# sqliteai/sqlite-vector

Hardware: AMD Instinct MI355X
Metric: vectors scanned/sec, L2 top-20 over Nx384 f32 (higher is better)
Workload: dtype f32; 1 GPU; 10Mx384 f32 L2 top-20 single-query; rows_per_gpu=10000000, dim=384, k=20, backend=HIP gfx950 x1

## Files before the change

### sqlite-vector_amd/csrc/vg_corpus.hip

```cpp
#include "vg_internal.h"

#include <atomic>
#include <mutex>
#include <utility>
#include <vector>

#include "vg_device.h"


static thread_local std::string g_err;

int vg_fail(int code, const char *fmt, ...) {
    char buf[1024];
    va_list ap;
    va_start(ap, fmt);
    vsnprintf(buf, sizeof(buf), fmt, ap);
    va_end(ap);
    g_err = buf;
    return code;
}

extern "C" const char *vg_last_error(void) { return g_err.c_str(); }
extern "C" void vg_set_last_error_(const char *msg) { g_err = msg ? msg : ""; }

// ... 70 lines not shown
    {"VG_SHAPE_F16_ROUND3", 1},
    {"VG_SHAPE_INT_SHORT_ROUND3", 1},
    {"VG_SHAPE_PREF_ROUND1", 1},
    {"VG_U", 1},
};
std::atomic<int> vg_switch_values[VGSW_COUNT];
void vg_switches_read(void) {
    for (int i = 0; i < VGSW_COUNT; ++i) {
        int v = VGSW_UNSET;
#ifndef VG_LAB
        if (!vg_switch_names[i].lab)
#endif
        {
            const char *e = getenv(vg_switch_names[i].name);
            if (e && *e) {
                if (i == SW_VG_SCAN_FILTER_SHADOW) v = (unsigned char)e[0];
                else if (i == SW_VECTORGPU_SHARD_GATHER) v = (e[0] == 'r' || e[0] == 'R') ? 1 : 0;
                else v = atoi(e);
            }
        }
        vg_switch_values[i].store(v, std::memory_order_relaxed);
    }
}
__attribute__((constructor)) static void vg_switches_at_load(void) { vg_switches_read(); }
extern "C" void vg_reload_switches(void) { vg_switches_read(); }

extern "C" int vg_corpus_create(int device, int vtype, int dim, int64_t capacity_rows_hint, vg_corpus **out) {
    if (!out) return vg_fail(VG_ERR_INVALID, "vg_corpus_create: out is NULL");
    *out = nullptr;
    vg_switches_read();
    int es = vg_elem_size(vtype);
// ... 739 lines not shown
```

### sqlite-vector_amd/csrc/vg_filter.hip

```cpp
#include "vg_internal.h"

#include "vg_scan.h"
#include "vg_scan_filter.h"
#include "vg_scan_filter_n4.h"

typedef VgShape Shape;

typedef void (*filter_fn_t)(FilterScanArgs);

static bool scan_filter_enabled(const vg_corpus *c) {
    if (c->filter_disabled) return false;
    if (c->scan_filter_mode >= 0) return c->scan_filter_mode != 0;
    return vg_sw(SW_VG_SCAN_FILTER, 1) != 0;
}
bool vg_scan_filter_policy(const vg_corpus *c) {
    return scan_filter_enabled(c) && c->n_rows * c->stride >= (long long)vg_sw(SW_VG_SCAN_FILTER_MIN_MB, 3072) * (1ll << 20);
}
bool vg_scan_filter_would_serve(const vg_corpus *c, int metric, int k);
int vg_ensure_filter_counters(vg_corpus *c) {
    if (c->d_filter_evals) return VG_OK;
    HIP_TRY(hipMalloc(&c->d_filter_evals, 4 * sizeof(unsigned long long)));
    HIP_TRY(hipMemsetAsync(c->d_filter_evals, 0, 4 * sizeof(unsigned long long), c->stream));
    HIP_TRY(hipHostMalloc(&c->h_filter_evals, 4 * sizeof(unsigned long long)));
    c->h_filter_evals[0] = c->h_filter_evals[1] = c->h_filter_evals[2] = c->h_filter_evals[3] = 0;
// ... 11 lines not shown
    }
    if (vg_sw(SW_VG_SCAN_FILTER_MIN_MB, -1) >= 0) return c->n_rows * c->stride >= (long long)vg_sw(SW_VG_SCAN_FILTER_MIN_MB, 0) * (1ll << 20);
    return c->n_rows >= (1 << 20) && c->n_rows * c->stride >= (768ll << 20);
}
static bool scan_filter_serves(const vg_corpus *c, int metric) {
    if (c->vtype == VG_TYPE_U8 || c->vtype == VG_TYPE_I8) return scan_filter_serves_n4(c, metric);
    const bool half = (c->vtype == VG_TYPE_F16 || c->vtype == VG_TYPE_BF16);
    if (c->vtype != VG_TYPE_F32 && !half) return false;
    if (metric == VG_DIST_L1 && !half) return false;
    if (metric != VG_DIST_L2 && metric != VG_DIST_SQUARED_L2 && metric != VG_DIST_DOT && metric != VG_DIST_COSINE && metric != VG_DIST_L1) return false;
    if (half && metric == VG_DIST_COSINE && !vg_sw(SW_VG_HALF_COSN, 1)) return false;
    if (!scan_filter_enabled(c)) return false;
    if (filter_uses_q8(c, metric) && vg_sw(SW_VG_SCAN_FILTER_MIN_MB, -1) < 0)
        return c->n_rows >= (1 << 20) && c->n_rows * c->stride >= (512ll << 20);
    return c->n_rows * c->stride >= (long long)vg_sw(SW_VG_SCAN_FILTER_MIN_MB, half ? 1024 : 3072) * (1ll << 20);
}

template <int XT, int MODE, bool NT, bool Q8>
static filter_fn_t pick_filter_u(int U) {
    switch (U) {
        case 1: return vg_scan_filter_kernel<XT, MODE, 1, NT, Q8>;
        case 2: return vg_scan_filter_kernel<XT, MODE, 2, NT, Q8>;
        case 3: return vg_scan_filter_kernel<XT, MODE, 3, NT, Q8>;
        case 4: return vg_scan_filter_kernel<XT, MODE, 4, NT, Q8>;
        case 6: return vg_scan_filter_kernel<XT, MODE, 6, NT, Q8>;
    }
    return nullptr;
}
template <int XT, bool NT, bool Q8>
static filter_fn_t pick_filter_mode(int mode, int U) {
// ... 149 lines not shown
            float ex = sx * sqrtf(e2);
            ex = ex * (1.0f + 4.0e-6f) + 1.0e-37f;
            stat[r] = bad ? make_float2(__builtin_nanf(""), 0.0f) : make_float2(sx, e2 > 0.0f ? ex : 0.0f);
        }
    }
}
typedef void (*to_q8_fn_t)(const uint8_t *, long long, long long, long long, int, int, uint8_t *, long long, float2 *);
template <int XT> static to_q8_fn_t pick_to_q8_reg(int nch) {
    if (nch <= 32) return vg_to_q8_reg_kernel<XT, 2>;
    if (nch <= 64) return vg_to_q8_reg_kernel<XT, 4>;
    if (nch <= 96) return vg_to_q8_reg_kernel<XT, 6>;
    if (nch <= 128) return vg_to_q8_reg_kernel<XT, 8>;
    return nullptr;
}

template <int XT, int MODE, bool NT>
static filter_fn_t pick_n4_u(int U) {
    switch (U) {
        case 1: return vg_scan_filter_n4_kernel<XT, MODE, 1, NT>;
        case 2: return vg_scan_filter_n4_kernel<XT, MODE, 2, NT>;
        case 3: return vg_scan_filter_n4_kernel<XT, MODE, 3, NT>;
        case 4: return vg_scan_filter_n4_kernel<XT, MODE, 4, NT>;
        case 6: return vg_scan_filter_n4_kernel<XT, MODE, 6, NT>;
    }
    return nullptr;
}
template <bool NT>
static filter_fn_t pick_n4(int vtype, int mode, int U) {
    if (vtype == VG_TYPE_U8) return mode == VGF_L2 ? pick_n4_u<T_U8, VGF_L2, NT>(U) : (mode == VGF_DOT ? pick_n4_u<T_U8, VGF_DOT, NT>(U) : pick_n4_u<T_U8, VGF_COS, NT>(U));
    return mode == VGF_L2 ? pick_n4_u<T_I8, VGF_L2, NT>(U) : (mode == VGF_DOT ? pick_n4_u<T_I8, VGF_DOT, NT>(U) : pick_n4_u<T_I8, VGF_COS, NT>(U));
}
static long long n4_shadow_stride(const vg_corpus *c) { return (((long long)c->dim + 31) / 32) * 16; }
int vg_ensure_n4_shadow(vg_corpus *c, int64_t upto_rows) {
    const long long ns = n4_shadow_stride(c);
    upto_rows = std::min<int64_t>(upto_rows, c->n_rows);
    if (c->n4_cap < upto_rows) {
        const int64_t cap = (upto_rows < c->n_rows) ? upto_rows : std::max<int64_t>(c->cap_rows, c->n_rows);
        HIP_TRY(hipStreamSynchronize(c->stream));
        if (c->d_rows_n4) hipFree(c->d_rows_n4);
        if (c->d_n4stat) hipFree(c->d_n4stat);
        c->d_rows_n4 = nullptr; c->d_n4stat = nullptr; c->n4_cap = 0; c->n4_rows = 0;
        if (hipMalloc(&c->d_rows_n4, (size_t)cap * ns) != hipSuccess || hipMalloc(&c->d_n4stat, (size_t)cap * sizeof(VgN4Stat)) != hipSuccess) {
            (void)hipGetLastError();
            if (c->d_rows_n4) hipFree(c->d_rows_n4);
            if (c->d_n4stat) hipFree(c->d_n4stat);
            c->d_rows_n4 = nullptr; c->d_n4stat = nullptr;
            return vg_fail(VG_ERR_NOMEM, "no device memory for the high-nibble shadow copy (%lld rows)", (long long)cap);
        }
        c->n4_cap = cap;
    }
    upto_rows = std::min<int64_t>(upto_rows, c->n_rows);
    if (c->n4_rows < upto_rows) {
        const long long n = upto_rows - c->n4_rows;
        const long long blocks = std::min<long long>((n * 16 + 255) / 256, 256 * 32);
        auto kern = c->vtype == VG_TYPE_U8 ? vg_to_n4_kernel<T_U8> : vg_to_n4_kernel<T_I8>;
        hipLaunchKernelGGL(kern, dim3((unsigned)blocks), dim3(256), 0, c->stream, c->d_rows, (long long)c->n4_rows, n,
                           (long long)c->stride, c->dim, c->d_rows_n4, ns, reinterpret_cast<VgN4Stat *>(c->d_n4stat));
        hipError_t e = hipGetLastError();
        if (e != hipSuccess) return vg_fail(VG_ERR_HIP, "nibble shadow pass failed: %s", hipGetErrorString(e));
        c->n4_rows = upto_rows;
    }
    return VG_OK;
}

static long long q8_shadow_stride(const vg_corpus *c) { return (((long long)c->dim + 15) / 16) * 16; }
static bool filter_uses_q8(const vg_corpus *c, int metric) {
    if (c->vtype != VG_TYPE_F32 && c->vtype != VG_TYPE_F16 && c->vtype != VG_TYPE_BF16) return false;
    if (metric == VG_DIST_L1 || c->q8_disabled) return false;
    const int e = vg_sw(SW_VG_SCAN_FILTER_SHADOW, 0);
    return !(e == 'b' || e == 'B' || e == 'r' || e == 'R');
}
int vg_ensure_q8_shadow(vg_corpus *c) {
    const long long qs = q8_shadow_stride(c);
    if (c->q8_cap < c->n_rows) {
        const int64_t cap = std::max<int64_t>(c->cap_rows, c->n_rows);
        HIP_TRY(hipStreamSynchronize(c->stream));
        if (c->d_rows_q8) hipFree(c->d_rows_q8);
        if (c->d_q8stat) hipFree(c->d_q8stat);
        c->d_rows_q8 = nullptr; c->d_q8stat = nullptr; c->q8_cap = 0; c->q8_rows = 0;
        if (hipMalloc(&c->d_rows_q8, (size_t)cap * qs) != hipSuccess || hipMalloc(&c->d_q8stat, (size_t)cap * sizeof(float2)) != hipSuccess) {
            (void)hipGetLastError();
            if (c->d_rows_q8) hipFree(c->d_rows_q8);
            if (c->d_q8stat) hipFree(c->d_q8stat);
            c->d_rows_q8 = nullptr; c->d_q8stat = nullptr;
            return vg_fail(VG_ERR_NOMEM, "no device memory for the int8 shadow copy (%lld rows)", (long long)cap);
// ... 22 lines not shown
            c->pass_rows[2] = n;
            hipEventDestroy(e0); hipEventDestroy(e1);
        }
        hipError_t e = hipGetLastError();
        if (e != hipSuccess) return vg_fail(VG_ERR_HIP, "int8 shadow pass failed: %s", hipGetErrorString(e));
        c->q8_rows = c->n_rows;
    }
    return VG_OK;
}
static int filter_mode_of(int metric) {
    return (metric == VG_DIST_DOT) ? VGF_DOT : (metric == VG_DIST_COSINE ? VGF_COS : (metric == VG_DIST_L1 ? VGF_L1 : VGF_L2));
}
static int filter_u_cap(const vg_corpus *) { return 6; }
static long long filter_stream_stride(const vg_corpus *c, int metric) {
    if (c->vtype == VG_TYPE_U8 || c->vtype == VG_TYPE_I8) return n4_shadow_stride(c);
    if (filter_uses_q8(c, metric)) return q8_shadow_stride(c);
    return c->vtype == VG_TYPE_F32 ? vg_bf16_shadow_stride(c) : (long long)c->stride;
}

int vg_launch_scan_filter(vg_corpus *c, int metric, const uint8_t *dev_query, int k, uint64_t *dev_out_keys, hipStream_t stream,
                          bool ref_emit, uint64_t *final_out) {
    if (!scan_filter_serves(c, metric)) return -1;
    const bool f32 = (c->vtype == VG_TYPE_F32);
    const bool n4 = (c->vtype == VG_TYPE_U8 || c->vtype == VG_TYPE_I8);
    const bool probing = n4 && !n4_explicit(c) && c->n4_probe != 1;
    const int64_t scan_rows = probing ? std::min<int64_t>(c->n_rows, 1ll << 21) : c->n_rows;
    int rc = n4 ? VG_OK : vg_ensure_row_norms(c);
    bool q8 = filter_uses_q8(c, metric);
    if (n4) {
        rc = vg_ensure_n4_shadow(c, scan_rows);
        if (rc == VG_ERR_NOMEM) { (void)hipGetLastError(); c->n4_disabled = true; return -1; }
    } else if (rc == VG_OK && q8) {
        rc = vg_ensure_q8_shadow(c);
        if (rc == VG_ERR_NOMEM && !f32) { (void)hipGetLastError(); c->q8_disabled = true; q8 = false; rc = VG_OK; }
    } else if (rc == VG_OK && f32) rc = vg_ensure_bf16_shadow(c);
    if (rc == VG_ERR_NOMEM) {
        (void)hipGetLastError();
        c->filter_disabled = true;
        return -1;
    }
    if (rc != VG_OK) return rc;
    const long long bs = filter_stream_stride(c, metric);
    const int nch_b = (int)(bs / 16);
    Shape s;
    vg_choose_shape(nch_b, VG_TYPE_U8, A_DOT, &s, filter_u_cap(c));
    if (s.long_rows) return -1;
    {
        const int fl = vg_sw(SW_VG_FILTER_LPR_LOG2, -1), fu = vg_sw(SW_VG_FILTER_U, -1);
        if (fl >= 0 && fl <= 6 && fu > 0 && (nch_b + (1 << fl) - 1) / (1 << fl) <= fu &&
            (n4 ? pick_n4<true>(c->vtype, filter_mode_of(metric), fu) : pick_filter<true>(c->vtype, filter_mode_of(metric), fu, q8))) { s.lpr_log2 = fl; s.U = fu; }
    }
    Shape xs;
    vg_plain_scan_shape(c, metric, &xs);
    if (xs.long_rows) return -1;
    if ((rc = vg_ensure_filter_counters(c)) != VG_OK) return rc;
    {
        unsigned long long now = 0;
        long long landed = 0;
        for (int attempt = 0; attempt < 4; ++attempt) {
            landed = (long long)*(volatile unsigned long long *)(c->h_filter_evals + 2);
            now = *(volatile unsigned long long *)c->h_filter_evals;
            if (landed == (long long)*(volatile unsigned long long *)(c->h_filter_evals + 2)) break;
        }
        const long long launches = std::min<long long>(c->filter_launches, landed) - c->filter_launches_seen;
        if (launches >= 2) {
// ... 8 lines not shown
        if (c->filter_cooldown > 0 && !probing) { --c->filter_cooldown; return -1; }
    }
    unsigned long long evals_before = 0;
    if (probing) {
        HIP_TRY(hipStreamSynchronize(c->stream));
        HIP_TRY(hipMemcpy(&evals_before, c->d_filter_evals, sizeof(evals_before), hipMemcpyDeviceToHost));
    }
    if (stream != c->stream) {
        if (!c->norm_ev) HIP_TRY(hipEventCreateWithFlags(&c->norm_ev, hipEventDisableTiming));
        HIP_TRY(hipEventRecord(c->norm_ev, c->stream));
        HIP_TRY(hipStreamWaitEvent(stream, c->norm_ev, 0));
    }
    const bool nt = (vg_sw(SW_VG_NT, -1) >= 0) ? vg_sw(SW_VG_NT, -1) != 0 : (scan_rows * bs > (256ll << 20));
    const int mode = filter_mode_of(metric);
    filter_fn_t fn = n4 ? (nt ? pick_n4<true>(c->vtype, mode, s.U) : pick_n4<false>(c->vtype, mode, s.U))
                        : (nt ? pick_filter<true>(c->vtype, mode, s.U, q8) : pick_filter<false>(c->vtype, mode, s.U, q8));
    if (!fn) return -1;
    const int rpb = VG_WAVE >> s.lpr_log2;
    const long long nbatch = (scan_rows + rpb - 1) / rpb;
    long long blocks = (nbatch + VG_WAVES_PER_BLOCK - 1) / VG_WAVES_PER_BLOCK;
    blocks = std::max<long long>(1, std::min<long long>(blocks, (long long)c->cu_count));
    blocks = std::min<long long>(blocks, VG_SEL_MAX_HEADS);
    FilterScanArgs a{};
    a.shadow = n4 ? c->d_rows_n4 : (q8 ? c->d_rows_q8 : (f32 ? c->d_rows_bf : c->d_rows));
    a.q8stat = reinterpret_cast<const float2 *>(n4 ? c->d_n4stat : c->d_q8stat); a.rows = c->d_rows; a.query = dev_query; a.row_norm = c->d_xnorm; a.cand = c->d_cand;
    a.n_rows = scan_rows; a.stride = c->stride; a.bstride = bs; a.nch = c->nch; a.nch_b = nch_b;
    a.lpr_log2 = s.lpr_log2; a.k = k; a.root = (metric == VG_DIST_L2) ? 1 : 0; a.dim = c->dim;
    a.mode = mode;
    a.cerr = (float)(c->dim + 64) * 4.76837158203125e-7f + (f32 ? 0.0078125f + 1.52587890625e-5f : 0.0f);
#ifdef VG_TEST_ROUND1_CERR
    if (f32) a.cerr = 0.00390625f + 1.6e-5f + (float)(c->dim + 64) * 4.76837158203125e-7f;
#endif
    a.rel = (float)(c->dim + 64) * 2.384185791015625e-7f;
    a.xlpr_log2 = xs.lpr_log2; a.xU = xs.U;
    a.evals = c->d_filter_evals;
    const size_t smem = std::max<size_t>((size_t)c->nch * 16 + ((q8 && !f32) ? (size_t)nch_b * 64 : 0), (size_t)VG_PUBLISH_LDS_BYTES);
    if (c->append_pending && stream != c->stream) HIP_TRY(hipStreamWaitEvent(stream, c->append_ev, 0));
    const bool emitting = ref_emit && !probing && scan_rows >= VG_REF_EMIT_MIN_ROWS;
    const bool prepass = (vg_sw(SW_VG_SCAN_FILTER_PREPASS, 1) != 0 && scan_rows >= (1 << 20)) || emitting;
    hipEvent_t *evs = probing ? nullptr : vg_prof_slot(c, (uint8_t)(VG_EVF_MERGE | (prepass ? VG_EVF_PREPASS : 0)));
// ... 37 lines not shown
    if (smem > 64 * 1024) HIP_TRY(hipFuncSetAttribute(reinterpret_cast<const void *>(fn), hipFuncAttributeMaxDynamicSharedMemorySize, (int)smem));
    hipLaunchKernelGGL(fn, dim3((unsigned)blocks), dim3(VG_BLOCK), smem, stream, a);
    ++c->filter_launches;
    if (evs) hipEventRecord(evs[2], stream);
    const bool mirror_in_merge = !probing && vg_sw(SW_VG_SCAN_FILTER_MIRROR_COPY, 0) == 0;
    const int rcm = vg_launch_merge_one((const uint64_t *)c->d_cand, (int)blocks, k, (final_out && !probing) ? final_out : dev_out_keys, stream,
                                        mirror_in_merge ? c->d_filter_evals : nullptr, mirror_in_merge ? c->h_filter_evals : nullptr);
    if (evs) hipEventRecord(evs[3], stream);
    if (!mirror_in_merge) HIP_TRY(hipMemcpyAsync(c->h_filter_evals, c->d_filter_evals, 3 * sizeof(unsigned long long), hipMemcpyDeviceToHost, stream));
    if (rcm != 0) return vg_fail(VG_ERR_HIP, "merge launch failed: %s", hipGetErrorString((hipError_t)rcm));
    HIP_TRY(hipGetLastError());
    if (probing) {
        HIP_TRY(hipStreamSynchronize(stream));
        unsigned long long evals_after = 0;
        HIP_TRY(hipMemcpy(&evals_after, c->d_filter_evals, sizeof(evals_after), hipMemcpyDeviceToHost));
        const bool selective = (evals_after - evals_before) * 8ull < (unsigned long long)scan_rows;
        c->n4_probe = selective ? 1 : 2;
        c->n4_probe_rows = c->n_rows;
        c->filter_evals_seen = evals_after;
        c->filter_launches_seen = c->filter_launches;
        if (!selective) {
            hipFree(c->d_rows_n4); hipFree(c->d_n4stat);
            c->d_rows_n4 = nullptr; c->d_n4stat = nullptr; c->n4_rows = 0; c->n4_cap = 0;
        }
        return vg_launch_scan_filter(c, metric, dev_query, k, dev_out_keys, stream, ref_emit, final_out);
    }
    return VG_OK;
}

bool vg_scan_filter_would_serve(const vg_corpus *c, int metric, int k) {
    if (k > VG_MAX_FUSED_K || c->filter_cooldown > 0 || !scan_filter_serves(c, metric)) return false;
// ... 1 lines not shown
    return true;
}

static const char *filter_type_tag(int t) { return t == VG_TYPE_F32 ? "f32" : (t == VG_TYPE_F16 ? "f16" : (t == VG_TYPE_BF16 ? "bf16" : (t == VG_TYPE_U8 ? "u8" : "i8"))); }

bool vg_scan_filter_name(vg_corpus *c, int metric, char *out, size_t out_len) {
    if (!scan_filter_serves(c, metric)) return false;
    const long long bs = filter_stream_stride(c, metric);
    Shape fs, xs;
    vg_choose_shape((int)(bs / 16), VG_TYPE_U8, A_DOT, &fs, filter_u_cap(c));
    vg_plain_scan_shape(c, metric, &xs);
    if (fs.long_rows || xs.long_rows) return false;
    const bool nt = (vg_sw(SW_VG_NT, -1) >= 0) ? vg_sw(SW_VG_NT, -1) != 0 : (c->n_rows * bs > (256ll << 20));
    static const char *mtag[4] = {"l2", "dot", "cos", "l1"};
    snprintf(out, out_len, "scan_filter_%s_%s%s_u%d_lpr%d%s", filter_type_tag(c->vtype), mtag[filter_mode_of(metric)],
             (c->vtype == VG_TYPE_U8 || c->vtype == VG_TYPE_I8) ? "_n4" : (filter_uses_q8(c, metric) ? "_q8" : (c->vtype == VG_TYPE_F32 ? "_bf16" : "")),
             fs.U, 1 << fs.lpr_log2, nt ? "_nt" : "");
    return true;
}
```

### sqlite-vector_amd/csrc/vg_scan_filter.h

```cpp
#pragma once

#include "vg_scan.h"

struct FilterScanArgs {
    const uint8_t *shadow;
    const uint8_t *rows;
    const uint8_t *query;
    const float *row_norm;
    const float2 *q8stat;
    uint64_t *cand;
    long long n_rows, stride, bstride;
    int nch, nch_b;
    int lpr_log2, k, root, mode, dim;
    float cerr;
    float rel;
    int xlpr_log2, xU;
    const uint64_t *init_keys;
    const uint64_t *init_lists;
    int n_init_lists;
    unsigned long long *evals;
    unsigned long long *emit;
    unsigned emit_cap;
};
enum { VGF_L2 = 0, VGF_DOT = 1, VGF_COS = 2, VGF_L1 = 3  };

typedef __bf16 vgf_bf16x2 __attribute__((ext_vector_type(2)));

__device__ inline uint32_t vgf_pack_bf16(uint32_t lo, uint32_t hi) {
    return ((lo + 0x7FFFu + ((lo >> 16) & 1u)) >> 16) | ((hi + 0x7FFFu + ((hi >> 16) & 1u)) & 0xFFFF0000u);
}

template <int FT>
__device__ inline void vgf_dot_chunk(const uint4 &q, const uint4 &x, float &s0, float &s1) {
    if constexpr (FT == T_BF16) {
        s0 = __builtin_amdgcn_fdot2_f32_bf16(__builtin_bit_cast(vgf_bf16x2, q.x), __builtin_bit_cast(vgf_bf16x2, x.x), s0, false);
        s1 = __builtin_amdgcn_fdot2_f32_bf16(__builtin_bit_cast(vgf_bf16x2, q.y), __builtin_bit_cast(vgf_bf16x2, x.y), s1, false);
        s0 = __builtin_amdgcn_fdot2_f32_bf16(__builtin_bit_cast(vgf_bf16x2, q.z), __builtin_bit_cast(vgf_bf16x2, x.z), s0, false);
        s1 = __builtin_amdgcn_fdot2_f32_bf16(__builtin_bit_cast(vgf_bf16x2, q.w), __builtin_bit_cast(vgf_bf16x2, x.w), s1, false);
    } else {
        s0 = __builtin_amdgcn_fdot2(__builtin_bit_cast(vg_half2, q.x), __builtin_bit_cast(vg_half2, x.x), s0, false);
// ... 14 lines not shown
    return (int)fminf(fmaxf(t, -127.0f), 127.0f);
}
template <int FT>
__device__ inline void vgf_l1_chunk(const uint4 &q, const uint4 &x, float &s0, float &s1) {
    const uint32_t qw[4] = {q.x, q.y, q.z, q.w}, xw[4] = {x.x, x.y, x.z, x.w};
#pragma unroll
    for (int j = 0; j < 4; ++j) {
        float q0, q1, x0, x1;
        vg_unpack2<FT>(qw[j], q0, q1);
        vg_unpack2<FT>(xw[j], x0, x1);
        s0 += fabsf(q0 - x0);
        s1 += fabsf(q1 - x1);
    }
}

template <int XT, int MODE, int U, bool NT, bool Q8 = false>
__global__ __launch_bounds__(VG_BLOCK) void vg_scan_filter_kernel(FilterScanArgs a) {
    constexpr bool XF32 = (XT == T_F32);
    constexpr bool L1M = (MODE == VGF_L1);
    constexpr int mode = MODE;
    static_assert(!(XF32 && L1M), "the f32 L1 scan has no filter variant");
    constexpr int FT = XF32 ? T_BF16 : XT;
    extern __shared__ __attribute__((aligned(16))) uint8_t smem[];
    const int lane = threadIdx.x & (VG_WAVE - 1);
    const int wave = threadIdx.x >> 6;
    const int lpr_log2 = a.lpr_log2, lpr = 1 << lpr_log2, rpb = VG_WAVE >> lpr_log2;
    const int sub = lane & (lpr - 1), rib = lane >> lpr_log2;
    const int k = a.k;

    uint4 *qs = reinterpret_cast<uint4 *>(smem);
    for (int c = threadIdx.x; c < a.nch; c += VG_BLOCK) qs[c] = reinterpret_cast<const uint4 *>(a.query)[c];
    __syncthreads();
    float q8_sq = 0.0f, q8_sqi = 0.0f, q8_eqn = 0.0f;
    bool q8_ok = true;
    float q8_inv = 0.0f, q8_qq = 0.0f;
    const float *qf = reinterpret_cast<const float *>(smem);
    if constexpr (Q8) {
        const int nqf = 16 * a.nch_b;
        if constexpr (!XF32) {
            float *wq = reinterpret_cast<float *>(smem + (size_t)a.nch * 16);
            for (int e2 = threadIdx.x; e2 < nqf / 2; e2 += VG_BLOCK) {
                float lo = 0.0f, hi = 0.0f;
                if (e2 < a.nch * 4) vg_unpack2<XT>(reinterpret_cast<const uint32_t *>(smem)[e2], lo, hi);
                wq[2 * e2] = lo; wq[2 * e2 + 1] = hi;
            }
            __syncthreads();
            qf = wq;
        }
        const int nq_have = XF32 ? a.nch * 4 : nqf;
        float mx = 0.0f;
        uint32_t bad = 0;
        for (int e = lane; e < nq_have; e += VG_WAVE) { const float f = qf[e]; mx = fmaxf(mx, fabsf(f)); bad |= !(fabsf(f) <= 3.0e38f); }
        mx = fmaxf(mx, vg_dpp<VG_DPP_QUAD_PERM(1, 0, 3, 2)>(mx));
        mx = fmaxf(mx, vg_dpp<VG_DPP_QUAD_PERM(2, 3, 0, 1)>(mx));
        mx = fmaxf(mx, vg_dpp<VG_DPP_ROW_HALF_MIRROR>(mx));
        mx = fmaxf(mx, vg_dpp<VG_DPP_ROW_MIRROR>(mx));
        mx = fmaxf(mx, __shfl_xor(mx, 16));
        mx = fmaxf(mx, __shfl_xor(mx, 32));
        q8_ok = (__ballot(bad != 0) == 0) && mx >= 1.0e-30f && mx <= 1.0e30f;
        q8_sq = q8_ok ? mx / 127.0f : 1.0f;
        q8_inv = 1.0f / q8_sq;
        uint32_t i2 = 0;
        float e2s = 0.0f, q2s = 0.0f;
        for (int e = lane; e < nq_have; e += VG_WAVE) {
            const float f = qf[e];
            const int qi = vgf_q8(f, q8_inv);
            const float r = fmaf(-q8_sq, (float)qi, f);
            i2 += (uint32_t)(qi * qi);
            e2s = fmaf(r, r, e2s);
            q2s = fmaf(f, f, q2s);
        }
        i2 = vg_group_sum(i2, 6);
        e2s = vg_group_sum(e2s, 6);
        q8_qq = vg_group_sum(q2s, 6);
        q8_sqi = q8_sq * sqrtf((float)i2) * (1.0f + 1.0e-5f);
        q8_eqn = sqrtf(e2s) * (1.0f + 1.0e-4f);
    }
    uint4 q[U];
#pragma unroll
    for (int u = 0; u < U; ++u) {
        const int cb = sub + u * lpr;
        if constexpr (Q8) {
            const int have = XF32 ? a.nch * 4 : 16 * a.nch_b;
            uint32_t w[4];
#pragma unroll
            for (int j = 0; j < 4; ++j) {
                w[j] = 0u;
#pragma unroll
                for (int b4 = 0; b4 < 4; ++b4) {
                    const int e = 16 * cb + 4 * j + b4;
                    if (cb < a.nch_b && e < have) w[j] |= (uint32_t)(vgf_q8(qf[e], q8_inv) & 255) << (8 * b4);
                }
            }
            q[u] = make_uint4(w[0], w[1], w[2], w[3]);
        } else if constexpr (XF32) {
            const uint4 f0 = (2 * cb < a.nch) ? qs[2 * cb] : make_uint4(0u, 0u, 0u, 0u);
            const uint4 f1 = (2 * cb + 1 < a.nch) ? qs[2 * cb + 1] : make_uint4(0u, 0u, 0u, 0u);
// ... 74 lines not shown
        const float t2 = a.root ? t * t : t;
        return t2 * (1.0f + 2.0f * a.rel) + 1e-30f;
    };
    float gate_init = INFINITY;
    uint64_t emit_below = VG_EMPTY_KEY;
    if (a.init_lists || a.init_keys) {
        const uint64_t kk = a.init_lists ? vg_kth_head(a.init_lists, a.n_init_lists, k, smem + VG_PUBLISH_LDS_BYTES - VG_KTH_HEAD_SCRATCH_BYTES - 16)
                                         : a.init_keys[k - 1];
        if (kk != VG_EMPTY_KEY) { gate_init = gate_of(vg_sortable_f32((uint32_t)(kk >> 32))); emit_below = kk & 0xFFFFFFFF00000000ull; }
    }
    float thr_gate = gate_init;
    auto refresh_gate = [&]() {
        const float t = (thr == VG_EMPTY_KEY) ? INFINITY : vg_sortable_f32((uint32_t)(thr >> 32));
        thr_gate = fminf(gate_of(t), gate_init);
    };
    auto exact_with = [&](auto acc, uint32_t row_u) -> float {
        typedef decltype(acc) A;
        const uint8_t *rp = a.rows + (unsigned long long)row_u * (unsigned long long)a.stride;
        const uint4 *xp = reinterpret_cast<const uint4 *>(rp);
        acc.init();
        for (int u = 0; u < a.xU; ++u) { const int c = xs + u * xlpr; if (c < a.nch) acc.chunk(qs[c], xp[c]); else acc.chunk(zero4, zero4); }
        typename A::QStat st;
        float d;
        if constexpr (XF32) {
            st.qq = xq_f32;
            d = acc.finish(st, a.xlpr_log2, a.root);
        } else {
            st.qq = xq_f64; st.qspecial = xq_special;
            if constexpr (MODE == VGF_COS) d = acc.finish_cached_norm(st, a.xlpr_log2, a.row_norm[row_u]);
            else d = acc.finish(st, a.xlpr_log2, a.root);
            if (acc.special(st, a.xlpr_log2) && xs == 0) {
                const uint16_t *q16 = reinterpret_cast<const uint16_t *>(qs), *r16 = reinterpret_cast<const uint16_t *>(rp);
                constexpr int SLOW = L1M ? A_L1 : (MODE == VGF_L2 ? A_L2 : (MODE == VGF_DOT ? A_DOT : A_COS));
                d = vg_slow_distance<XT, SLOW>(q16, r16, a.dim, a.root);
            }
        }
        return vg_clamp(d);
    };
    auto exact = [&](uint32_t row_u) -> float {
        constexpr int XACC = L1M ? A_L1 : (MODE == VGF_L2 ? A_L2 : (MODE == VGF_DOT ? A_DOT : (XF32 ? A_COS : A_COSN)));
        return exact_with(Accum<XT, XACC>(), row_u);
    };

    const long long nbatch = (a.n_rows + rpb - 1) / rpb;
    const long long wstride = (long long)gridDim.x * VG_WAVES_PER_BLOCK;
    long long b = (long long)blockIdx.x * VG_WAVES_PER_BLOCK + wave;
    uint4 cur[U], nxt[U];
    float nrm_cur = 0.0f, nrm_nxt = 0.0f;
    float2 q8_cur = make_float2(0.0f, 0.0f), q8_nxt = make_float2(0.0f, 0.0f);
    auto load = [&](uint4 (&dst)[U], float &nrm, float2 &q8s, long long batch) {
        vg_load_batch<U, NT>(dst, a.shadow, batch * rpb + rib, (batch < nbatch) ? a.n_rows : 0, a.bstride, sub, lpr, a.nch_b);
        const long long r0 = batch * rpb + rib;
        const bool live = batch < nbatch && r0 < a.n_rows;
        const long long ri = live ? r0 : 0;
        const float nv = a.row_norm[ri];
        nrm = live ? nv : 0.0f;
        if constexpr (Q8) { const float2 qv = a.q8stat[ri]; q8s = live ? qv : make_float2(0.0f, 0.0f); }
    };
    load(cur, nrm_cur, q8_cur, b);
    while (b < nbatch) {
        const long long bn = b + wstride;
// ... 47 lines not shown
                ++n_exact;
                const uint64_t key = vg_make_key(de, row_u);
                if (de < INFINITY && key < thr) {
                    vg_list_insert(mine, thr, key, lane, k);
                    refresh_gate();
                    if (a.emit && key < emit_below) vg_emit_pair(a.emit, a.emit_cap, key, lane);
                }
            }
        }
#pragma unroll
        for (int u = 0; u < U; ++u) cur[u] = nxt[u];
        nrm_cur = nrm_nxt;
        q8_cur = q8_nxt;
        b = bn;
    }
    __syncthreads();
    if (a.evals) {
        unsigned *blk = reinterpret_cast<unsigned *>(smem + VG_PUBLISH_LDS_BYTES - sizeof(unsigned));
        if (threadIdx.x == 0) *blk = 0u;
        __syncthreads();
        if (lane == 0 && n_exact) atomicAdd(blk, n_exact);
        __syncthreads();
        if (threadIdx.x == 0 && *blk) atomicAdd(a.evals, (unsigned long long)*blk);
        if (threadIdx.x == 0 && blockIdx.x == 0) atomicAdd(a.evals + 2, 1ull);
        __syncthreads();
    }
    vg_block_publish(smem, mine, k, a.cand + (long long)blockIdx.x * VG_WAVE);
}
```

### sqlite-vector_amd/csrc/vg_switches.h

```cpp
#pragma once
#include <atomic>
#include <climits>

enum VgSwitch {
    SW_VECTORGPU_SHARD_GATHER,
    SW_VECTORGPU_SHARD_THREADS,
    SW_VG_BATCH_BPC,
    SW_VG_BATCH_H_SPLIT,
    SW_VG_BATCH_H_WAVES,
    SW_VG_BATCH_LONG,
    SW_VG_BATCH_LONG_BPC,
    SW_VG_BATCH_MFMA,
    SW_VG_BATCH_MIN_QUERIES,
    SW_VG_BATCH_PREPASS,
    SW_VG_BATCH_Q8,
    SW_VG_BATCH_SLICE,
    SW_VG_BATCH_STAGES,
    SW_VG_BATCH_TILE_MAJOR,
    SW_VG_BLOCKS_PER_CU,
    SW_VG_F32_FILTER,
    SW_VG_FILTER_LPR_LOG2,
    SW_VG_FILTER_U,
    SW_VG_FORCE_LONG,
    SW_VG_HALF_COSN,
// ... 14 lines not shown
    SW_VG_SCAN_FILTER_PREMERGE,
    SW_VG_SCAN_FILTER_PREPASS,
    SW_VG_SCAN_FILTER_PREPASS_DIV,
    SW_VG_SCAN_FILTER_SHADOW,
    SW_VG_SCAN_ORDER,
    SW_VG_SHAPE_BF16_L2_U3,
    SW_VG_SHAPE_F16_ROUND3,
    SW_VG_SHAPE_INT_SHORT_ROUND3,
    SW_VG_SHAPE_PREF_ROUND1,
    SW_VG_U,
    VGSW_COUNT
};
#define VGSW_UNSET INT_MIN
extern std::atomic<int> vg_switch_values[VGSW_COUNT];
void vg_switches_read(void);
static inline int vg_sw(VgSwitch id, int dflt) { const int v = vg_switch_values[id].load(std::memory_order_relaxed); return v == VGSW_UNSET ? dflt : v; }
static inline bool vg_sw_set(VgSwitch id) { return vg_switch_values[id].load(std::memory_order_relaxed) != VGSW_UNSET; }
```

Baseline: 4.439 billion vectors/s.

## Add 4-bit quantized shadow filter for f32 scans with probe-based selection

Adds a 4-bit (nibble) quantized shadow copy of f32 rows with per-row scale, residual norm and row norm, plus a filter kernel variant that computes bounds using sdot4 against the int8 query. Rows whose lower bound cannot beat the current top-k threshold are skipped, and survivors get an exact f32 distance. The q4 path cuts streamed bytes per row roughly in half compared with the q8 shadow, and uses a deeper multi-buffer load pipeline. A probe on the first rows decides whether q4 is selective enough to keep. The trade-off is looser bounds, which may send more rows to exact f32 re-evaluation, plus the cost of building the shadow copy and running the probe.

```diff
diff --git a/sqlite-vector_amd/csrc/vg_corpus.hip b/sqlite-vector_amd/csrc/vg_corpus.hip
--- a/sqlite-vector_amd/csrc/vg_corpus.hip
+++ b/sqlite-vector_amd/csrc/vg_corpus.hip
@@ -108,7 +108,8 @@
         {
             const char *e = getenv(vg_switch_names[i].name);
             if (e && *e) {
-                if (i == SW_VG_SCAN_FILTER_SHADOW) v = (unsigned char)e[0];
+                if (i == SW_VG_SCAN_FILTER_SHADOW)
+                    v = ((e[0] == 'q' || e[0] == 'Q') && e[1] == '4' && e[2] == 0) ? VG_SHADOW_Q4 : (unsigned char)e[0];
                 else if (i == SW_VECTORGPU_SHARD_GATHER) v = (e[0] == 'r' || e[0] == 'R') ? 1 : 0;
                 else v = atoi(e);
             }
diff --git a/sqlite-vector_amd/csrc/vg_filter.hip b/sqlite-vector_amd/csrc/vg_filter.hip
--- a/sqlite-vector_amd/csrc/vg_filter.hip
+++ b/sqlite-vector_amd/csrc/vg_filter.hip
@@ -49,6 +49,22 @@
     if (filter_uses_q8(c, metric) && vg_sw(SW_VG_SCAN_FILTER_MIN_MB, -1) < 0)
         return c->n_rows >= (1 << 20) && c->n_rows * c->stride >= (512ll << 20);
     return c->n_rows * c->stride >= (long long)vg_sw(SW_VG_SCAN_FILTER_MIN_MB, half ? 1024 : 3072) * (1ll << 20);
+}
+
+template <int MODE, bool NT>
+static filter_fn_t pick_q4_u(int U) {
+    switch (U) {
+        case 1: return vg_scan_filter_kernel<T_F32, MODE, 1, NT, true, true>;
+        case 2: return vg_scan_filter_kernel<T_F32, MODE, 2, NT, true, true>;
+        case 3: return vg_scan_filter_kernel<T_F32, MODE, 3, NT, true, true>;
+        case 4: return vg_scan_filter_kernel<T_F32, MODE, 4, NT, true, true>;
+        case 6: return vg_scan_filter_kernel<T_F32, MODE, 6, NT, true, true>;
+    }
+    return nullptr;
+}
+template <bool NT>
+static filter_fn_t pick_q4(int mode, int U) {
+    return mode == VGF_L2 ? pick_q4_u<VGF_L2, NT>(U) : (mode == VGF_DOT ? pick_q4_u<VGF_DOT, NT>(U) : (mode == VGF_COS ? pick_q4_u<VGF_COS, NT>(U) : nullptr));
 }
 
 template <int XT, int MODE, bool NT, bool Q8>
@@ -228,6 +244,83 @@
     return nullptr;
 }
 
+
+template <int U>
+__global__ __launch_bounds__(256) void vg_to_q4_reg_kernel(const uint8_t *rows, long long row0, long long n, long long stride, int dim,
+                                                           int nch, const float *xnorm, uint8_t *out, long long ostride, VgQ4Stat *stat) {
+    const int l16 = threadIdx.x & 15;
+    const long long groups = ((long long)gridDim.x * blockDim.x) >> 4;
+    const long long n_pad = ((n + 3) / 4) * 4;
+    for (long long i = ((long long)blockIdx.x * blockDim.x + threadIdx.x) >> 4; i < n_pad; i += groups) {
+        const bool live = i < n;
+        const long long r = row0 + (live ? i : n - 1);
+        const uint8_t *src = rows + r * stride;
+        uint4 raw[U];
+#pragma unroll
+        for (int u = 0; u < U; ++u) {
+            const int c = l16 + 16 * u;
+            raw[u] = vg_load16<true>(c < nch ? src + (long long)c * 16 : reinterpret_cast<const uint8_t *>(vg_zero_chunk));
+        }
+        float v[U][4];
+        float mx = 0.0f;
+        uint32_t bad = 0;
+#pragma unroll
+        for (int u = 0; u < U; ++u) {
+            const int c = l16 + 16 * u;
+            const uint32_t w[4] = {raw[u].x, raw[u].y, raw[u].z, raw[u].w};
+#pragma unroll
+            for (int j = 0; j < 4; ++j) {
+                v[u][j] = (c * 4 + j < dim) ? __uint_as_float(w[j]) : 0.0f;
+                const float av = fabsf(v[u][j]);
+                mx = fmaxf(mx, av);
+                bad |= !(av <= 3.0e38f) ? 1u : 0u;
+            }
+        }
+        mx = fmaxf(mx, vg_dpp<VG_DPP_QUAD_PERM(1, 0, 3, 2)>(mx));
+        mx = fmaxf(mx, vg_dpp<VG_DPP_QUAD_PERM(2, 3, 0, 1)>(mx));
+        mx = fmaxf(mx, vg_dpp<VG_DPP_ROW_HALF_MIRROR>(mx));
+        mx = fmaxf(mx, vg_dpp<VG_DPP_ROW_MIRROR>(mx));
+        bad = vg_group_or(bad, 4);
+        const float sx = (mx > 0.0f) ? mx / 7.0f : 0.0f;
+        const float inv = (mx > 0.0f) ? 1.0f / sx : 0.0f;
+        if (!(fabsf(inv) <= 3.0e38f)) bad = 1u;
+        double e2 = 0.0;
+        uint8_t *o = out + r * ostride;
+#pragma unroll
+        for (int u = 0; u < U; ++u) {
+            const int c = l16 + 16 * u;
+            uint32_t p = 0;
+#pragma unroll
+            for (int j = 0; j < 4; ++j) {
+                const float x = v[u][j];
+                const float tq = bad ? 0.0f : fminf(fmaxf(rintf(x * inv), -7.0f), 7.0f);
+                const int xi = (int)tq;
+                const double res = bad ? 0.0 : (double)x - (double)sx * (double)xi;
+                e2 += res * res;
+                p |= (uint32_t)(xi + 8) << (8 * j);
+            }
+            const uint32_t pn = vg_dpp<VG_DPP_QUAD_PERM(1, 0, 3, 2)>(p);
+            if (live && !(l16 & 1) && 2 * c < (int)ostride) *reinterpret_cast<uint32_t *>(o + 2 * c) = p | (pn << 4);
+        }
+        e2 = vg_group_sum(e2, 4);
+        if (live && l16 == 0) {
+            float ex = (float)sqrt(e2);
+            ex = ex * (1.0f + 4.0e-7f) + 1.0e-37f;
+            VgQ4Stat s;
+            s.sx = bad ? __builtin_nanf("") : sx; s.exn = (bad || !(e2 > 0.0)) ? 0.0f : ex; s.xn = xnorm[r]; s.spare = 0u;
+            stat[r] = s;
+        }
+    }
+}
+typedef void (*to_q4_fn_t)(const uint8_t *, long long, long long, long long, int, int, const float *, uint8_t *, long long, VgQ4Stat *);
+static to_q4_fn_t pick_to_q4_reg(int nch) {
+    if (nch <= 32) return vg_to_q4_reg_kernel<2>;
+    if (nch <= 64) return vg_to_q4_reg_kernel<4>;
+    if (nch <= 96) return vg_to_q4_reg_kernel<6>;
+    if (nch <= 128) return vg_to_q4_reg_kernel<8>;
+    return nullptr;
+}
+
 template <int XT, int MODE, bool NT>
 static filter_fn_t pick_n4_u(int U) {
     switch (U) {
@@ -244,6 +337,9 @@
     if (vtype == VG_TYPE_U8) return mode == VGF_L2 ? pick_n4_u<T_U8, VGF_L2, NT>(U) : (mode == VGF_DOT ? pick_n4_u<T_U8, VGF_DOT, NT>(U) : pick_n4_u<T_U8, VGF_COS, NT>(U));
     return mode == VGF_L2 ? pick_n4_u<T_I8, VGF_L2, NT>(U) : (mode == VGF_DOT ? pick_n4_u<T_I8, VGF_DOT, NT>(U) : pick_n4_u<T_I8, VGF_COS, NT>(U));
 }
+#ifndef VG_Q4_PROBE_DIV
+#define VG_Q4_PROBE_DIV 8
+#endif
 static long long n4_shadow_stride(const vg_corpus *c) { return (((long long)c->dim + 31) / 32) * 16; }
 int vg_ensure_n4_shadow(vg_corpus *c, int64_t upto_rows) {
     const long long ns = n4_shadow_stride(c);
@@ -259,7 +355,7 @@
             if (c->d_rows_n4) hipFree(c->d_rows_n4);
             if (c->d_n4stat) hipFree(c->d_n4stat);
             c->d_rows_n4 = nullptr; c->d_n4stat = nullptr;
-            return vg_fail(VG_ERR_NOMEM, "no device memory for the high-nibble shadow copy (%lld rows)", (long long)cap);
+            return vg_fail(VG_ERR_NOMEM, "no device memory for the nibble shadow copy (%lld rows)", (long long)cap);
         }
         c->n4_cap = cap;
     }
@@ -267,9 +363,16 @@
     if (c->n4_rows < upto_rows) {
         const long long n = upto_rows - c->n4_rows;
         const long long blocks = std::min<long long>((n * 16 + 255) / 256, 256 * 32);
+        if (c->vtype == VG_TYPE_F32) {
+            to_q4_fn_t q4k = pick_to_q4_reg(c->nch);
+            if (!q4k || c->xnorm_rows < upto_rows) return vg_fail(VG_ERR_INVALID, "4-bit shadow pass: row norms missing or rows too long");
+            hipLaunchKernelGGL(q4k, dim3((unsigned)blocks), dim3(256), 0, c->stream, c->d_rows, (long long)c->n4_rows, n,
+                               (long long)c->stride, c->dim, c->nch, c->d_xnorm, c->d_rows_n4, ns, reinterpret_cast<VgQ4Stat *>(c->d_n4stat));
+        } else {
         auto kern = c->vtype == VG_TYPE_U8 ? vg_to_n4_kernel<T_U8> : vg_to_n4_kernel<T_I8>;
         hipLaunchKernelGGL(kern, dim3((unsigned)blocks), dim3(256), 0, c->stream, c->d_rows, (long long)c->n4_rows, n,
                            (long long)c->stride, c->dim, c->d_rows_n4, ns, reinterpret_cast<VgN4Stat *>(c->d_n4stat));
+        }
         hipError_t e = hipGetLastError();
         if (e != hipSuccess) return vg_fail(VG_ERR_HIP, "nibble shadow pass failed: %s", hipGetErrorString(e));
         c->n4_rows = upto_rows;
@@ -283,6 +386,18 @@
     if (metric == VG_DIST_L1 || c->q8_disabled) return false;
     const int e = vg_sw(SW_VG_SCAN_FILTER_SHADOW, 0);
     return !(e == 'b' || e == 'B' || e == 'r' || e == 'R');
+}
+static bool q4_eligible(const vg_corpus *c, int metric) {
+    return c->vtype == VG_TYPE_F32 && metric != VG_DIST_L1 && !c->q8_disabled && !c->n4_disabled && c->nch <= 128;
+}
+static bool q4_forced(const vg_corpus *c, int metric) { return q4_eligible(c, metric) && vg_sw(SW_VG_SCAN_FILTER_SHADOW, 0) == VG_SHADOW_Q4; }
+static bool q4_wants_probe(const vg_corpus *c, int metric) {
+    if (!q4_eligible(c, metric) || vg_sw_set(SW_VG_SCAN_FILTER_SHADOW)) return false;
+    return c->n4_probe == 0 || (c->n4_probe == 2 && c->n_rows >= 2 * c->n4_probe_rows);
+}
+static bool filter_uses_q4(const vg_corpus *c, int metric) {
+    if (q4_forced(c, metric)) return true;
+    return q4_eligible(c, metric) && !vg_sw_set(SW_VG_SCAN_FILTER_SHADOW) && c->n4_probe == 1;
 }
 int vg_ensure_q8_shadow(vg_corpus *c) {
     const long long qs = q8_shadow_stride(c);
@@ -335,6 +450,7 @@
 static int filter_u_cap(const vg_corpus *) { return 6; }
 static long long filter_stream_stride(const vg_corpus *c, int metric) {
     if (c->vtype == VG_TYPE_U8 || c->vtype == VG_TYPE_I8) return n4_shadow_stride(c);
+    if (filter_uses_q4(c, metric)) return n4_shadow_stride(c);
     if (filter_uses_q8(c, metric)) return q8_shadow_stride(c);
     return c->vtype == VG_TYPE_F32 ? vg_bf16_shadow_stride(c) : (long long)c->stride;
 }
@@ -344,13 +460,21 @@
     if (!scan_filter_serves(c, metric)) return -1;
     const bool f32 = (c->vtype == VG_TYPE_F32);
     const bool n4 = (c->vtype == VG_TYPE_U8 || c->vtype == VG_TYPE_I8);
-    const bool probing = n4 && !n4_explicit(c) && c->n4_probe != 1;
+    const bool q4_probing = !n4 && !ref_emit && filter_uses_q8(c, metric) && q4_wants_probe(c, metric);
+    const bool probing = (n4 && !n4_explicit(c) && c->n4_probe != 1) || q4_probing;
     const int64_t scan_rows = probing ? std::min<int64_t>(c->n_rows, 1ll << 21) : c->n_rows;
     int rc = n4 ? VG_OK : vg_ensure_row_norms(c);
     bool q8 = filter_uses_q8(c, metric);
+    const bool q4 = !n4 && !ref_emit && q8 && (q4_probing || filter_uses_q4(c, metric));
     if (n4) {
         rc = vg_ensure_n4_shadow(c, scan_rows);
         if (rc == VG_ERR_NOMEM) { (void)hipGetLastError(); c->n4_disabled = true; return -1; }
+    } else if (rc == VG_OK && q4) {
+        rc = vg_ensure_n4_shadow(c, scan_rows);
+        if (rc == VG_ERR_NOMEM) {
+            (void)hipGetLastError(); c->n4_disabled = true;
+            return vg_launch_scan_filter(c, metric, dev_query, k, dev_out_keys, stream, ref_emit, final_out);
+        }
     } else if (rc == VG_OK && q8) {
         rc = vg_ensure_q8_shadow(c);
         if (rc == VG_ERR_NOMEM && !f32) { (void)hipGetLastError(); c->q8_disabled = true; q8 = false; rc = VG_OK; }
@@ -361,7 +485,7 @@
         return -1;
     }
     if (rc != VG_OK) return rc;
-    const long long bs = filter_stream_stride(c, metric);
+    const long long bs = (n4 || q4) ? n4_shadow_stride(c) : (q8 ? q8_shadow_stride(c) : (f32 ? vg_bf16_shadow_stride(c) : (long long)c->stride));
     const int nch_b = (int)(bs / 16);
     Shape s;
     vg_choose_shape(nch_b, VG_TYPE_U8, A_DOT, &s, filter_u_cap(c));
@@ -369,7 +493,7 @@
     {
         const int fl = vg_sw(SW_VG_FILTER_LPR_LOG2, -1), fu = vg_sw(SW_VG_FILTER_U, -1);
         if (fl >= 0 && fl <= 6 && fu > 0 && (nch_b + (1 << fl) - 1) / (1 << fl) <= fu &&
-            (n4 ? pick_n4<true>(c->vtype, filter_mode_of(metric), fu) : pick_filter<true>(c->vtype, filter_mode_of(metric), fu, q8))) { s.lpr_log2 = fl; s.U = fu; }
+            (n4 ? pick_n4<true>(c->vtype, filter_mode_of(metric), fu) : (q4 ? pick_q4<true>(filter_mode_of(metric), fu) : pick_filter<true>(c->vtype, filter_mode_of(metric), fu, q8)))) { s.lpr_log2 = fl; s.U = fu; }
     }
     Shape xs;
     vg_plain_scan_shape(c, metric, &xs);
@@ -408,6 +532,7 @@
     const bool nt = (vg_sw(SW_VG_NT, -1) >= 0) ? vg_sw(SW_VG_NT, -1) != 0 : (scan_rows * bs > (256ll << 20));
     const int mode = filter_mode_of(metric);
     filter_fn_t fn = n4 ? (nt ? pick_n4<true>(c->vtype, mode, s.U) : pick_n4<false>(c->vtype, mode, s.U))
+                   : q4 ? (nt ? pick_q4<true>(mode, s.U) : pick_q4<false>(mode, s.U))
                         : (nt ? pick_filter<true>(c->vtype, mode, s.U, q8) : pick_filter<false>(c->vtype, mode, s.U, q8));
     if (!fn) return -1;
     const int rpb = VG_WAVE >> s.lpr_log2;
@@ -416,8 +541,8 @@
     blocks = std::max<long long>(1, std::min<long long>(blocks, (long long)c->cu_count));
     blocks = std::min<long long>(blocks, VG_SEL_MAX_HEADS);
     FilterScanArgs a{};
-    a.shadow = n4 ? c->d_rows_n4 : (q8 ? c->d_rows_q8 : (f32 ? c->d_rows_bf : c->d_rows));
-    a.q8stat = reinterpret_cast<const float2 *>(n4 ? c->d_n4stat : c->d_q8stat); a.rows = c->d_rows; a.query = dev_query; a.row_norm = c->d_xnorm; a.cand = c->d_cand;
+    a.shadow = (n4 || q4) ? c->d_rows_n4 : (q8 ? c->d_rows_q8 : (f32 ? c->d_rows_bf : c->d_rows));
+    a.q8stat = reinterpret_cast<const float2 *>((n4 || q4) ? c->d_n4stat : c->d_q8stat); a.rows = c->d_rows; a.query = dev_query; a.row_norm = c->d_xnorm; a.cand = c->d_cand;
     a.n_rows = scan_rows; a.stride = c->stride; a.bstride = bs; a.nch = c->nch; a.nch_b = nch_b;
     a.lpr_log2 = s.lpr_log2; a.k = k; a.root = (metric == VG_DIST_L2) ? 1 : 0; a.dim = c->dim;
     a.mode = mode;
@@ -485,7 +610,7 @@
         HIP_TRY(hipStreamSynchronize(stream));
         unsigned long long evals_after = 0;
         HIP_TRY(hipMemcpy(&evals_after, c->d_filter_evals, sizeof(evals_after), hipMemcpyDeviceToHost));
-        const bool selective = (evals_after - evals_before) * 8ull < (unsigned long long)scan_rows;
+        const bool selective = (evals_after - evals_before) * (q4_probing ? (unsigned long long)VG_Q4_PROBE_DIV : 8ull) < (unsigned long long)scan_rows;
         c->n4_probe = selective ? 1 : 2;
         c->n4_probe_rows = c->n_rows;
         c->filter_evals_seen = evals_after;
@@ -517,7 +642,7 @@
     const bool nt = (vg_sw(SW_VG_NT, -1) >= 0) ? vg_sw(SW_VG_NT, -1) != 0 : (c->n_rows * bs > (256ll << 20));
     static const char *mtag[4] = {"l2", "dot", "cos", "l1"};
     snprintf(out, out_len, "scan_filter_%s_%s%s_u%d_lpr%d%s", filter_type_tag(c->vtype), mtag[filter_mode_of(metric)],
-             (c->vtype == VG_TYPE_U8 || c->vtype == VG_TYPE_I8) ? "_n4" : (filter_uses_q8(c, metric) ? "_q8" : (c->vtype == VG_TYPE_F32 ? "_bf16" : "")),
+             (c->vtype == VG_TYPE_U8 || c->vtype == VG_TYPE_I8 || filter_uses_q4(c, metric)) ? "_n4" : (filter_uses_q8(c, metric) ? "_q8" : (c->vtype == VG_TYPE_F32 ? "_bf16" : "")),
              fs.U, 1 << fs.lpr_log2, nt ? "_nt" : "");
     return true;
 }
diff --git a/sqlite-vector_amd/csrc/vg_scan_filter.h b/sqlite-vector_amd/csrc/vg_scan_filter.h
--- a/sqlite-vector_amd/csrc/vg_scan_filter.h
+++ b/sqlite-vector_amd/csrc/vg_scan_filter.h
@@ -24,6 +24,8 @@
 };
 enum { VGF_L2 = 0, VGF_DOT = 1, VGF_COS = 2, VGF_L1 = 3  };
 
+struct VgQ4Stat { float sx, exn, xn; uint32_t spare; };
+
 typedef __bf16 vgf_bf16x2 __attribute__((ext_vector_type(2)));
 
 __device__ inline uint32_t vgf_pack_bf16(uint32_t lo, uint32_t hi) {
@@ -68,9 +70,10 @@
     }
 }
 
-template <int XT, int MODE, int U, bool NT, bool Q8 = false>
+template <int XT, int MODE, int U, bool NT, bool Q8 = false, bool Q4 = false>
 __global__ __launch_bounds__(VG_BLOCK) void vg_scan_filter_kernel(FilterScanArgs a) {
     constexpr bool XF32 = (XT == T_F32);
+    static_assert(!Q4 || (Q8 && XT == T_F32), "the 4-bit shadow copy: f32 corpora, with the int8 split of the query");
     constexpr bool L1M = (MODE == VGF_L1);
     constexpr int mode = MODE;
     static_assert(!(XF32 && L1M), "the f32 L1 scan has no filter variant");
@@ -88,6 +91,7 @@
     float q8_sq = 0.0f, q8_sqi = 0.0f, q8_eqn = 0.0f;
     bool q8_ok = true;
     float q8_inv = 0.0f, q8_qq = 0.0f;
+    int q4_bias = 0;
     const float *qf = reinterpret_cast<const float *>(smem);
     if constexpr (Q8) {
         const int nqf = 16 * a.nch_b;
@@ -114,27 +118,45 @@
         q8_ok = (__ballot(bad != 0) == 0) && mx >= 1.0e-30f && mx <= 1.0e30f;
         q8_sq = q8_ok ? mx / 127.0f : 1.0f;
         q8_inv = 1.0f / q8_sq;
-        uint32_t i2 = 0;
+        uint32_t i2 = 0, i1s = 0;
         float e2s = 0.0f, q2s = 0.0f;
         for (int e = lane; e < nq_have; e += VG_WAVE) {
             const float f = qf[e];
             const int qi = vgf_q8(f, q8_inv);
             const float r = fmaf(-q8_sq, (float)qi, f);
             i2 += (uint32_t)(qi * qi);
+            if constexpr (Q4) i1s += (uint32_t)qi;
             e2s = fmaf(r, r, e2s);
             q2s = fmaf(f, f, q2s);
         }
         i2 = vg_group_sum(i2, 6);
+        if constexpr (Q4) q4_bias = 8 * (int)vg_group_sum(i1s, 6);
         e2s = vg_group_sum(e2s, 6);
         q8_qq = vg_group_sum(q2s, 6);
         q8_sqi = q8_sq * sqrtf((float)i2) * (1.0f + 1.0e-5f);
         q8_eqn = sqrtf(e2s) * (1.0f + 1.0e-4f);
     }
     uint4 q[U];
+    uint4 qh[Q4 ? U : 1];
+    (void)qh;
 #pragma unroll
     for (int u = 0; u < U; ++u) {
         const int cb = sub + u * lpr;
-        if constexpr (Q8) {
+        if constexpr (Q4) {
+            const int have = a.nch * 4;
+            uint32_t w[8];
+#pragma unroll
+            for (int j = 0; j < 8; ++j) {
+                w[j] = 0u;
+#pragma unroll
+                for (int b4 = 0; b4 < 4; ++b4) {
+                    const int e = 32 * cb + 4 * j + b4;
+                    if (cb < a.nch_b && e < have) w[j] |= (uint32_t)(vgf_q8(qf[e], q8_inv) & 255) << (8 * b4);
+                }
+            }
+            q[u] = make_uint4(w[0], w[1], w[2], w[3]);
+            qh[u] = make_uint4(w[4], w[5], w[6], w[7]);
+        } else if constexpr (Q8) {
             const int have = XF32 ? a.nch * 4 : 16 * a.nch_b;
             uint32_t w[4];
 #pragma unroll
@@ -239,7 +261,7 @@
         const float t = (thr == VG_EMPTY_KEY) ? INFINITY : vg_sortable_f32((uint32_t)(thr >> 32));
         thr_gate = fminf(gate_of(t), gate_init);
     };
-    auto exact_with = [&](auto acc, uint32_t row_u) -> float {
+    auto exact_with = [&](auto acc, uint32_t row_u) __attribute__((always_inline)) -> float {
         typedef decltype(acc) A;
         const uint8_t *rp = a.rows + (unsigned long long)row_u * (unsigned long long)a.stride;
         const uint4 *xp = reinterpret_cast<const uint4 *>(rp);
@@ -262,7 +284,7 @@
         }
         return vg_clamp(d);
     };
-    auto exact = [&](uint32_t row_u) -> float {
+    auto exact = [&](uint32_t row_u) __attribute__((always_inline)) -> float {
         constexpr int XACC = L1M ? A_L1 : (MODE == VGF_L2 ? A_L2 : (MODE == VGF_DOT ? A_DOT : (XF32 ? A_COS : A_COSN)));
         return exact_with(Accum<XT, XACC>(), row_u);
     };
@@ -270,6 +292,79 @@
     const long long nbatch = (a.n_rows + rpb - 1) / rpb;
     const long long wstride = (long long)gridDim.x * VG_WAVES_PER_BLOCK;
     long long b = (long long)blockIdx.x * VG_WAVES_PER_BLOCK + wave;
+    if constexpr (Q4) {
+        constexpr int NB = (U <= 2) ? 4 : (U == 3 ? 3 : 2);
+        uint4 buf[NB][U];
+        uint4 rec[NB];
+        const VgQ4Stat *stats = reinterpret_cast<const VgQ4Stat *>(a.q8stat);
+        auto load4 = [&](uint4 (&dst)[U], uint4 &rs, long long batch) __attribute__((always_inline)) {
+            vg_load_batch<U, NT>(dst, a.shadow, batch * rpb + rib, (batch < nbatch) ? a.n_rows : 0, a.bstride, sub, lpr, a.nch_b);
+            const long long r0 = batch * rpb + rib;
+            const bool live = batch < nbatch && r0 < a.n_rows;
+            const uint4 rv = *reinterpret_cast<const uint4 *>(stats + (live ? r0 : 0));
+            rs = live ? rv : zero4;
+        };
+        auto process4 = [&](const uint4 (&cur)[U], const uint4 &rs, long long bcur) __attribute__((always_inline)) {
+            int i0 = 0, i1 = 0;
+#pragma unroll
+            for (int u = 0; u < U; ++u) {
+                const uint32_t w[4] = {cur[u].x, cur[u].y, cur[u].z, cur[u].w};
+                const uint32_t ql[4] = {q[u].x, q[u].z, qh[u].x, qh[u].z}, qu[4] = {q[u].y, q[u].w, qh[u].y, qh[u].w};
+#pragma unroll
+                for (int j = 0; j < 4; ++j) {
+                    i0 = __builtin_amdgcn_sdot4((int)ql[j], (int)(w[j] & 0x0F0F0F0Fu), i0, false);
+                    i1 = __builtin_amdgcn_sdot4((int)qu[j], (int)((w[j] >> 4) & 0x0F0F0F0Fu), i1, false);
+                }
+            }
+            const float sx = __uint_as_float(rs.x), exn = __uint_as_float(rs.y), nrm = __uint_as_float(rs.z);
+            const float st = (float)((int)vg_group_sum((uint32_t)(i0 + i1), lpr_log2) - q4_bias) * (q8_sq * sx);
+            const long long row = bcur * rpb + rib;
+            const float nn = nrm * nrm;
+            const float E = q8_sqi * exn + q8_eqn * nrm * (1.0f + a.rel) + 4.0e-7f * fabsf(st);
+            const bool zero_row = (nn == 0.0f);
+            const bool judged = q_ok && (zero_row || ((nrm >= 1.0e-15f && nrm <= 1.0e15f) && (sx > 0.0f && sx <= 3.0e38f)));
+            float lb;
+            if (mode == VGF_L2) lb = qq + nn - 2.0f * (st + E) - a.rel * (qq + nn);
+            else if (mode == VGF_DOT) lb = -(st + E) - a.rel * qn * nrm;
+            else { const float r = (st + E) / (qn * nrm); lb = zero_row ? 1.0f - 4.0e-6f : 1.0f - r - a.rel * fabsf(r) - 4.0e-6f; }
+            const bool cand = (sub == 0) && (row < a.n_rows) && (!judged || lb < thr_gate);
+            unsigned long long m = __ballot(cand);
+            while (m) {
+                const int ngrp = VG_WAVE >> a.xlpr_log2, gid = lane >> a.xlpr_log2;
+                int mysrc = __ffsll((long long)m) - 1, ntake = 0;
+                for (; ntake < ngrp && m; ++ntake) {
+                    const int s1 = __ffsll((long long)m) - 1;
+                    m &= m - 1;
+                    if (gid == ntake) mysrc = s1;
+                }
+                const uint32_t row_g = (uint32_t)__shfl((int)(uint32_t)row, mysrc);
+                const float d_g = exact(row_g);
+                for (int i = 0; i < ntake; ++i) {
+                    const int leader = i << a.xlpr_log2;
+                    const float de = __builtin_bit_cast(float, __builtin_amdgcn_readlane(__builtin_bit_cast(int, d_g), leader));
+                    const uint32_t row_u = (uint32_t)__builtin_amdgcn_readlane((int)row_g, leader);
+                    ++n_exact;
+                    const uint64_t key = vg_make_key(de, row_u);
+                    if (de < INFINITY && key < thr) {
+                        vg_list_insert(mine, thr, key, lane, k);
+                        refresh_gate();
+                        if (a.emit && key < emit_below) vg_emit_pair(a.emit, a.emit_cap, key, lane);
+                    }
+                }
+            }
+        };
+#pragma unroll
+        for (int j = 0; j < NB - 1; ++j) load4(buf[j], rec[j], b + j * wstride);
+        while (b < nbatch) {
+#pragma unroll
+            for (int j = 0; j < NB; ++j) {
+                const long long bj = b + j * wstride;
+                load4(buf[(j + NB - 1) % NB], rec[(j + NB - 1) % NB], bj + (NB - 1) * wstride);
+                if (bj < nbatch) process4(buf[j], rec[j], bj);
+            }
+            b += NB * wstride;
+        }
+    } else {
     uint4 cur[U], nxt[U];
     float nrm_cur = 0.0f, nrm_nxt = 0.0f;
     float2 q8_cur = make_float2(0.0f, 0.0f), q8_nxt = make_float2(0.0f, 0.0f);
@@ -347,6 +442,7 @@
         q8_cur = q8_nxt;
         b = bn;
     }
+    }
     __syncthreads();
     if (a.evals) {
         unsigned *blk = reinterpret_cast<unsigned *>(smem + VG_PUBLISH_LDS_BYTES - sizeof(unsigned));
diff --git a/sqlite-vector_amd/csrc/vg_switches.h b/sqlite-vector_amd/csrc/vg_switches.h
--- a/sqlite-vector_amd/csrc/vg_switches.h
+++ b/sqlite-vector_amd/csrc/vg_switches.h
@@ -52,5 +52,6 @@
 #define VGSW_UNSET INT_MIN
 extern std::atomic<int> vg_switch_values[VGSW_COUNT];
 void vg_switches_read(void);
+#define VG_SHADOW_Q4 0x3471
 static inline int vg_sw(VgSwitch id, int dflt) { const int v = vg_switch_values[id].load(std::memory_order_relaxed); return v == VGSW_UNSET ? dflt : v; }
 static inline bool vg_sw_set(VgSwitch id) { return vg_switch_values[id].load(std::memory_order_relaxed) != VGSW_UNSET; }
```

Result: no change. 4.436 billion vectors/s (-0.1%).
